# gareth-cross/mini_opt

Measured on AMD Instinct MI355X. Metric: batched dense KKT Newton steps/sec, n=64 fp64, higher is better.
Workload: dtype f64; 1 GPU; BASELINE configs[2]: batch=65536 per GPU, n=64 / 8 eq / 32 box, m_r=128, J-level input (row-major J), one mo_newton_step launch per step; mode=step, kernel=fused_mfma_f64_n64, batch_per_gpu=65536, batch_total=65536, n=64, k=8, m=32, m_r=128, parallelism=batch-sharded x1, no collectives

## Files before the change

### mini_opt_amd/csrc/kkt_fused.hip

```cpp
#include <math.h>
#include <stdlib.h>

#include <type_traits>

#include "mo_fused_device.h"
#include "mo_fused_diag.h"
#include "mo_fused_select.h"

namespace mo {
namespace {

typedef double d2 __attribute__((ext_vector_type(2)));
typedef double d4 __attribute__((ext_vector_type(4)));

constexpr int kRC = 15;

__device__ inline double readlane_f64(double v, int lane) {
  int lo = __double2loint(v), hi = __double2hiint(v);
  lo = __builtin_amdgcn_readlane(lo, lane);
  hi = __builtin_amdgcn_readlane(hi, lane);
  return __hiloint2double(hi, lo);
}
__device__ inline double bpermute_f64(int byte_addr, double v) {
  int lo = __builtin_amdgcn_ds_bpermute(byte_addr, __double2loint(v));
  int hi = __builtin_amdgcn_ds_bpermute(byte_addr, __double2hiint(v));
  return __hiloint2double(hi, lo);
}
typedef unsigned u2v __attribute__((ext_vector_type(2)));
template <int CTRL> __device__ inline double dpp_f64(double v) {
  int lo = __double2loint(v), hi = __double2hiint(v);
  lo = __builtin_amdgcn_mov_dpp(lo, CTRL, 0xf, 0xf, false);
  hi = __builtin_amdgcn_mov_dpp(hi, CTRL, 0xf, 0xf, false);
  return __hiloint2double(hi, lo);
}
__device__ inline double row_sum(double v) {
  v += dpp_f64<0xB1>(v);
  v += dpp_f64<0x4E>(v);
  v += dpp_f64<0x141>(v);
  v += dpp_f64<0x140>(v);
  return v;
}
__device__ inline int select_lanes32(unsigned long long mask, int if_set, int if_clear) {
  int r;
  asm("v_cndmask_b32 %0, %1, %2, %3" : "=v"(r) : "v"(if_clear), "v"(if_set), "s"(mask));
  return r;
}
__device__ inline double select_lanes(unsigned long long mask, double if_set, double if_clear) {
  return __hiloint2double(select_lanes32(mask, __double2hiint(if_set), __double2hiint(if_clear)),
                          select_lanes32(mask, __double2loint(if_set), __double2loint(if_clear)));
}
template <int CTRL, unsigned long long MASK> __device__ inline double exchange_add(double a, double b) {
  const double keep = select_lanes(MASK, b, a), send = select_lanes(MASK, a, b);
  return keep + dpp_f64<CTRL>(send);
}
__device__ inline double row_sum4_scatter(double p0, double p1, double p2, double p3) {
  const double q01 = exchange_add<0xB1, 0xAAAAAAAAAAAAAAAAull>(p0, p1);
  const double q23 = exchange_add<0xB1, 0xAAAAAAAAAAAAAAAAull>(p2, p3);
  double w = exchange_add<0x4E, 0xCCCCCCCCCCCCCCCCull>(q01, q23);
  w += dpp_f64<0x124>(w);
  w += dpp_f64<0x128>(w);
  return w;
}
__device__ inline double row_min(double v) {
  v = fmin(v, dpp_f64<0xB1>(v));
  v = fmin(v, dpp_f64<0x4E>(v));
  v = fmin(v, dpp_f64<0x141>(v));
  v = fmin(v, dpp_f64<0x140>(v));
  return v;
}
struct Rows2 { double a, b; };
__device__ inline Rows2 swap16_f64(double v) {
  const u2v lo = __builtin_amdgcn_permlane16_swap((unsigned)__double2loint(v), (unsigned)__double2loint(v), false, false);
  const u2v hi = __builtin_amdgcn_permlane16_swap((unsigned)__double2hiint(v), (unsigned)__double2hiint(v), false, false);
  return Rows2{__hiloint2double((int)hi[0], (int)lo[0]), __hiloint2double((int)hi[1], (int)lo[1])};
}
__device__ inline Rows2 swap32_f64(double v) {
  const u2v lo = __builtin_amdgcn_permlane32_swap((unsigned)__double2loint(v), (unsigned)__double2loint(v), false, false);
  const u2v hi = __builtin_amdgcn_permlane32_swap((unsigned)__double2hiint(v), (unsigned)__double2hiint(v), false, false);
  return Rows2{__hiloint2double((int)hi[0], (int)lo[0]), __hiloint2double((int)hi[1], (int)lo[1])};
}
__device__ inline double cross_row_sum(double v) {
  const Rows2 p = swap16_f64(v);
  const double s = p.a + p.b;
  const Rows2 q = swap32_f64(s);
  return q.a + q.b;
}
__device__ inline double cross_row_min(double v) {
  const Rows2 p = swap16_f64(v);
  const double s = fmin(p.a, p.b);
  const Rows2 q = swap32_f64(s);
  return fmin(q.a, q.b);
}
__device__ inline double rcp_f64(double d) {
  double q = __builtin_amdgcn_rcp(d);
  q = fma(q, fma(-d, q, 1.0), q);
  q = fma(q, fma(-d, q, 1.0), q);
  return q;
}
__device__ inline d4 mfma4(const d4& a, const d4& b, d4 c) {
  c = __builtin_amdgcn_mfma_f64_16x16x4f64(a[0], b[0], c, 0, 0, 0);
  c = __builtin_amdgcn_mfma_f64_16x16x4f64(a[1], b[1], c, 0, 0, 0);
  c = __builtin_amdgcn_mfma_f64_16x16x4f64(a[2], b[2], c, 0, 0, 0);
  c = __builtin_amdgcn_mfma_f64_16x16x4f64(a[3], b[3], c, 0, 0, 0);
  return c;
}

template <int NT, bool QPL> __device__ inline void ldv(const double* arr, int j, double (&v)[NT]) {
  if (QPL) {
#pragma unroll
    for (int c = 0; c < NT; ++c) v[c] = arr[16 * c + j];
  } else {
#pragma unroll
    for (int h = 0; h < NT / 2; ++h) { const d2 t = *(const d2*)(arr + 32 * h + 2 * j); v[2 * h] = t[0]; v[2 * h + 1] = t[1]; }
  }
}
template <int NT, bool QPL> __device__ inline void stv(double* arr, int j, const double (&v)[NT]) {
  if (QPL) {
#pragma unroll
    for (int c = 0; c < NT; ++c) arr[16 * c + j] = v[c];
  } else {
#pragma unroll
    for (int h = 0; h < NT / 2; ++h) { d2 t; t[0] = v[2 * h]; t[1] = v[2 * h + 1]; *(d2*)(arr + 32 * h + 2 * j) = t; }
  }
}
template <int NT, bool QPL> __device__ inline void ldv_n(const double* arr, int j, int nn, double (&v)[NT]) {
  if (QPL) {
#pragma unroll
    for (int c = 0; c < NT; ++c) v[c] = (16 * c + j < nn) ? arr[16 * c + j] : 0.0;
  } else {
#pragma unroll
    for (int h = 0; h < NT / 2; ++h) {
      v[2 * h] = (32 * h + 2 * j < nn) ? arr[32 * h + 2 * j] : 0.0;
      v[2 * h + 1] = (32 * h + 2 * j + 1 < nn) ? arr[32 * h + 2 * j + 1] : 0.0;
    }
  }
}
template <int NT, bool QPL> __device__ inline void stv_n(double* arr, int j, int nn, const double (&v)[NT]) {
  if (QPL) {
#pragma unroll
    for (int c = 0; c < NT; ++c)
      if (16 * c + j < nn) arr[16 * c + j] = v[c];
  } else {
#pragma unroll
    for (int h = 0; h < NT / 2; ++h) {
      if (32 * h + 2 * j < nn) arr[32 * h + 2 * j] = v[2 * h];
      if (32 * h + 2 * j + 1 < nn) arr[32 * h + 2 * j + 1] = v[2 * h + 1];
    }
  }
}
template <int NT, bool QPL> __device__ inline void pad_diag(int j, int nn, double (&v)[NT]) {
#pragma unroll
  for (int c = 0; c < NT; ++c) {
    const int nat = QPL ? 16 * c + j : 32 * (c >> 1) + 2 * j + (c & 1);
    v[c] = nat >= nn ? 1.0 : 0.0;
  }
}
template <int NT, bool QPL, int NY = 1>
__device__ inline void load_a_tiles(const double* Ap, int A_ld, int k, int nn, int g, int j, d4 (&U)[(NT + NY) * (NT + NY)]) {
  constexpr int NB = NT + NY;
  const int col_l = (QPL ? 1 : 2) * g;
  const double* Al = Ap + j + (size_t)col_l * A_ld;
#pragma unroll
  for (int c = 0; c < NT; ++c) {
#pragma unroll
    for (int t = 0; t < 4; ++t) {
      const int col_u = QPL ? (16 * c + 4 * t) : (32 * (c >> 1) + 8 * t + (c & 1));
#pragma unroll
      for (int q = 0; q < NY; ++q)
        U[c * NB + NT + q][t] = (16 * q + j < k && col_u + col_l < nn) ? Al[16 * q + (size_t)col_u * A_ld] : 0.0;
    }
  }
}
template <int NT, int NY = 1>
__device__ inline void load_g_tiles(const double* G, int ld, const double* cg, int nn, int g, int j, d4 (&U)[(NT + NY) * (NT + NY)],
                                    double (&cvec)[NT]) {
  constexpr int NB = NT + NY;
#pragma unroll
  for (int ta = 0; ta < NT; ++ta) {
#pragma unroll
    for (int tb = ta; tb < NT; ++tb) {
#pragma unroll
      for (int t = 0; t < 4; ++t) {
        const int r = g + 4 * t;
        int row = 16 * tb + j, col = 16 * ta + r;
        if (ta == tb && r > j) { row = 16 * ta + r; col = 16 * ta + j; }
        U[ta * NB + tb][t] = (row < nn && col < nn) ? G[row + (size_t)col * ld] : 0.0;
      }
    }
    cvec[ta] = (16 * ta + j < nn) ? cg[16 * ta + j] : 0.0;
  }
}

__device__ inline const void* uniform_ptr(const void* p) {
  return (const void*)(uintptr_t)uniform64((unsigned long long)(uintptr_t)p);
}
template <int IMM> __device__ inline void dma16_s(const void* sbase_in, unsigned voff, unsigned lds_dst_in) {
  const void* sbase = uniform_ptr(sbase_in);
  const unsigned lds_dst = __builtin_amdgcn_readfirstlane(lds_dst_in);
  unsigned keep;
  asm volatile(
      "s_mov_b32 %0, m0\n\ts_mov_b32 m0, %3\n\ts_nop 0\n\tglobal_load_lds_dwordx4 %1, %2 offset:%4 nt\n\ts_mov_b32 m0, %0"
      : "=&s"(keep)
      : "v"(voff), "s"(sbase), "s"(lds_dst), "i"(IMM)
      : "memory");
}
__device__ inline void dma4_s(const void* sbase_in, unsigned voff, unsigned lds_dst_in) {
  const void* sbase = uniform_ptr(sbase_in);
  const unsigned lds_dst = __builtin_amdgcn_readfirstlane(lds_dst_in);
  unsigned keep;
  asm volatile(
      "s_mov_b32 %0, m0\n\ts_mov_b32 m0, %3\n\ts_nop 0\n\tglobal_load_lds_dword %1, %2\n\ts_mov_b32 m0, %0"
      : "=&s"(keep)
      : "v"(voff), "s"(sbase), "s"(lds_dst)
      : "memory");
}
__device__ inline void dma_doubles(const double* src, unsigned lds_dst, int count, int lane) {
  const unsigned voff = 4u * (unsigned)lane;
  if (lane < 2 * count) dma4_s(src, voff, lds_dst);
  if (lane + 64 < 2 * count) dma4_s(reinterpret_cast<const char*>(src) + 256, voff, lds_dst + 256);
  if (count > 64) {
    if (lane + 128 < 2 * count) dma4_s(reinterpret_cast<const char*>(src) + 512, voff, lds_dst + 512);
    if (lane + 192 < 2 * count) dma4_s(reinterpret_cast<const char*>(src) + 768, voff, lds_dst + 768);
  }
  if (count > 128) {
#pragma unroll
    for (int c = 4; c < 8; ++c)
      if (lane + 64 * c < 2 * count) dma4_s(reinterpret_cast<const char*>(src) + 256 * c, voff, lds_dst + 256 * c);
  }
}

template <int LANE_IN_ROW> __device__ inline double row_bcast64(double v) {
  return __longlong_as_double(__builtin_amdgcn_mov_dpp(__double_as_longlong(v), 0x150 + LANE_IN_ROW, 0xf, 0xf, false));
}
template <unsigned long long MASK> __device__ inline void masked_set(double& dst, double src) {
  unsigned long long save;
  asm volatile("s_mov_b64 %[sv], exec\n\ts_mov_b32 exec_lo, %[lo]\n\ts_mov_b32 exec_hi, %[hi]\n\tv_mov_b64 %[d], %[s]\n\t"
               "s_mov_b64 exec, %[sv]\n\ts_nop 0"
               : [d] "+v"(dst), [sv] "=&s"(save)
               : [s] "v"(src), [lo] "i"((unsigned)(MASK & 0xffffffffull)), [hi] "i"((unsigned)(MASK >> 32)));
}
template <unsigned long long MASK> __device__ inline void masked_set_neg(double& dst, double src) {
  unsigned long long save;
  asm volatile("s_mov_b64 %[sv], exec\n\ts_mov_b32 exec_lo, %[lo]\n\ts_mov_b32 exec_hi, %[hi]\n\tv_max_f64 %[d], -%[s], -%[s]\n\t"
               "s_mov_b64 exec, %[sv]\n\ts_nop 0"
               : [d] "+v"(dst), [sv] "=&s"(save)
               : [s] "v"(src), [lo] "i"((unsigned)(MASK & 0xffffffffull)), [hi] "i"((unsigned)(MASK >> 32)));
}
template <unsigned long long MASK> __device__ inline void masked_zero4(d4& T) {
  unsigned long long save;
  double t0 = T[0], t1 = T[1], t2 = T[2], t3 = T[3];
  asm volatile(
      "s_mov_b64 %[sv], exec\n\ts_mov_b32 exec_lo, %[lo]\n\ts_mov_b32 exec_hi, %[hi]\n\tv_mov_b64 %[a], 0\n\tv_mov_b64 %[b], 0\n\t"
      "v_mov_b64 %[c], 0\n\tv_mov_b64 %[d], 0\n\ts_mov_b64 exec, %[sv]\n\ts_nop 0"
      : [a] "+v"(t0), [b] "+v"(t1), [c] "+v"(t2), [d] "+v"(t3), [sv] "=&s"(save)
      : [lo] "i"((unsigned)(MASK & 0xffffffffull)), [hi] "i"((unsigned)(MASK >> 32)));
  T[0] = t0; T[1] = t1; T[2] = t2; T[3] = t3;
}
template <int K>
__device__ inline void sweep_step_lean(d4& T, double& bad, int g, int j) {
  constexpr int src_g = K & 3, src_t = K >> 2;
  constexpr unsigned long long mcol = 0x0001000100010001ull << K;
  constexpr unsigned long long mrow = 0xFFFFull << (16 * src_g);
  const double rowreg = T[src_t];
  const double d = readlane_f64(rowreg, 16 * src_g + K);
  double inv = __builtin_amdgcn_rcp(d);
  inv = fma(inv, fma(-d, inv, 1.0), inv);
  asm volatile("v_fma_f64 %0, %1, 0, %0" : "+v"(bad) : "v"(inv));
  double rk = bpermute_f64((16 * src_g + j) * 4, rowreg) * inv;
  masked_set_neg<mcol>(rk, inv);
  double f[4];
#pragma unroll
  for (int t = 0; t < 4; ++t) f[t] = row_bcast64<K>(T[t]);
  masked_zero4<mcol>(T);
#pragma unroll
  for (int t = 0; t < 4; ++t) T[t] = fma(-f[t], rk, T[t]);
  double rowk_new = T[src_t];
  masked_set<mrow>(rowk_new, rk);
  T[src_t] = rowk_new;
}
template <int K, int KEND> struct SweepLoop {
  static __device__ inline void run(d4& T, double& bad, int npiv, int g, int j) {
    if (K < npiv) sweep_step_lean<K>(T, bad, g, j);
    SweepLoop<K + 1, KEND>::run(T, bad, npiv, g, j);
  }
};
template <int KEND> struct SweepLoop<KEND, KEND> {
  static __device__ inline void run(d4&, double&, int, int, int) {}
};
__device__ inline bool sweep_tile(d4& T, int npiv, int g, int j) {
  double bad = 0.0;
  SweepLoop<0, 16>::run(T, bad, npiv, g, j);
  return bad == 0.0;
}

template <int NT, int D, int JMODE = JMODE_VECTOR, int NY = 1, bool ROW0 = true, bool DIAG4 = false>
struct JStream {
  static constexpr bool FLAT = JMODE == JMODE_FLAT, GATHER = JMODE == JMODE_GATHER;
  static_assert(!DIAG4 || (JMODE == JMODE_VECTOR && NY == 1 && NT == 4), "DIAG4: the 16-byte stream of the 64 grid with one y tile");
  static constexpr int N = 16 * NT, NB = NT + NY, NH = NT / 2, NI = GATHER ? 2 * NT : (FLAT ? N / 8 : NH), DPS = NI + 1, SLOT = NH * 1024 + 64;
  static_assert((D - 1) * DPS <= 63, "vmcnt is a 6-bit counter");
  static_assert(D >= 2 && D <= 8, "ring depth");
  const char* jbase;
  const char* rbase;
  unsigned joff, roff;
  unsigned jstep;
  const double* tail_j; const double* tail_r; int rem, row_len, g_, j_;
  bool act0, act1, act2, act3;
  const char* lane_piece;
  const char* r_elem;
  const char* dop[DIAG4 ? diag4::kNumVec : 1];
  double dacc[DIAG4 ? NT / 2 : 1][diag4::kNumIns];
  unsigned ring_base;
  int lane, nsteps;
  long long rs_, cs_;

  __device__ inline void init(const double* Jp, const double* rg, const char* smem, unsigned ring_base_, int lane_, int g, int j, int m_r,
                              int nn = N, long long rs = -1, long long cs = 1) {
    if (rs < 0) rs = nn;
    jbase = reinterpret_cast<const char*>(Jp);
    rbase = reinterpret_cast<const char*>(rg);
    rs_ = 8 * rs; cs_ = 8 * cs;
    joff = GATHER ? (unsigned)(g * rs_ + 2 * j * cs_) : (unsigned)(g * nn + 2 * j) * 8u;
    jstep = GATHER ? (unsigned)(4 * rs_) : 32u * (unsigned)nn;
    act0 = 2 * j < nn; act1 = 32 + 2 * j < nn; act2 = 64 + 2 * j < nn; act3 = 96 + 2 * j < nn;
    roff = 4u * (unsigned)lane_;
    lane_piece = smem + lane_ * 16;
    if (DIAG4) {
      const int jp = diag4::swz(g, j);
      joff = (unsigned)(g * nn + 2 * jp) * 8u;
      act0 = 2 * jp < nn; act1 = 32 + 2 * jp < nn; act2 = 64 + 2 * jp < nn; act3 = 96 + 2 * jp < nn;
      lane_piece = smem + diag4::natural_off(lane_);
    }
    r_elem = smem + NH * 1024 + 8 * g;
    ring_base = ring_base_; lane = lane_; nsteps = m_r >> 2;
    rem = m_r & 3; row_len = nn; g_ = g; j_ = j;
    tail_j = Jp + (size_t)(4 * nsteps) * (GATHER ? rs : (long long)nn); tail_r = rg + 4 * nsteps;
  }
  template <int IMM> __device__ static inline void dma4_si(const void* sbase_in, unsigned voff, unsigned lds_dst_in) {
    const void* sbase = uniform_ptr(sbase_in);
    const unsigned lds_dst = __builtin_amdgcn_readfirstlane(lds_dst_in);
// ... 387 lines not shown
#pragma unroll
      for (int pb = pa + 1; pb < NB; ++pb) {
        double q2 = 0.0;
#pragma unroll
        for (int t = 0; t < 4; ++t) q2 = fma(U[pa * NB + pb][t], wr[t], q2);
        rb[pb] += cross_row_sum(q2);
        if constexpr (NY >= 2) asm volatile("" : "+v"(rb[pb]));
      }
      lds_fence();
    }
  }
#pragma unroll
  for (int pa = L; pa >= 0; --pa) {
    const double* rsrc = pa < NT ? rbuf_x + 16 * pa : rbuf_y + 16 * (pa - NT);
    double vt[4], pt[4];
#pragma unroll
    for (int t = 0; t < 4; ++t) {
      pt[t] = 0.0;
#pragma unroll
      for (int pb = pa + 1; pb < NB; ++pb) pt[t] = fma(U[pa * NB + pb][t], xb[pb], pt[t]);
    }
    if (pa < L) {
      const double ws = row_sum4_scatter(pt[0], pt[1], pt[2], pt[3]);
      pt[0] = row_bcast64<0>(ws); pt[1] = row_bcast64<1>(ws); pt[2] = row_bcast64<2>(ws); pt[3] = row_bcast64<3>(ws);
    }
#pragma unroll
    for (int t = 0; t < 4; ++t) vt[t] = rsrc[g + 4 * t] - pt[t];
    double q = 0.0;
#pragma unroll
    for (int t = 0; t < 4; ++t) q = fma(U[pa * NB + pa][t], vt[t], q);
    xb[pa] = -cross_row_sum(q);
    if (pa >= NT) xb[pa] = (16 * (pa - NT) + j < k) ? xb[pa] : 0.0;
    __builtin_amdgcn_sched_barrier(0);
  }
}

template <int NT, int WPS, int MC = 1, int NY = 1, bool RHS = false> struct FusedCfg {
  static constexpr int N = 16 * NT;
  static constexpr int NH = NT / 2;
  static constexpr int DPS = NH + 1;
  static constexpr int SLOT = NH * 1024 + 64;
  static constexpr int MCAP = 64 * MC;
  static constexpr int VEC = (3 * N + 4 * MCAP + MCAP / 2 + 32 * NY + (RHS ? MCAP : 0)) * 8;
  static constexpr int D_FIT = ((160 * 1024) / (4 * WPS) - VEC) / SLOT;
  static constexpr int D_TUNED = NT > 4 ? 4 : (NT == 4 ? (WPS >= 3 ? 4 : 7) : (WPS >= 4 ? 4 : 8));
  static constexpr int D = MC == 1 ? D_TUNED : (D_FIT > 8 ? 8 : D_FIT);
  static_assert(D >= 2, "LDS budget");
  static constexpr int LDS = D * SLOT + VEC;
};

template <int NT, int WPS, bool QPL, int MC = 1, int JMODE = JMODE_VECTOR, int NY = 1, bool RHS = false>
__global__ __launch_bounds__(256 * WPS, WPS) void kkt_fused_f64_kernel(const KernelArgs a) {
  static_assert(!RHS || JMODE == JMODE_VECTOR, "the right-hand-side mode exists on the 16-byte stream and for (G, c) only");
  using C = FusedCfg<NT, WPS, MC, NY, RHS>;
  constexpr int MCAP = C::MCAP;
  constexpr int N = C::N, NB = NT + NY, LT = NB - 1, SLOT = C::SLOT, D = C::D;
  constexpr int WAVES = 4 * WPS;

  __shared__ __attribute__((aligned(16))) char smem_all[WAVES * C::LDS];
  const int wave = __builtin_amdgcn_readfirstlane((int)(threadIdx.x >> 6));
  char* const smem = smem_all + wave * C::LDS;
  double* const xs = reinterpret_cast<double*>(smem + D * SLOT);
  double* const diagS = xs + N;
  double* const rhsS = diagS + N;
  double* const rp = diagS;
  double* const dxs = rhsS;
  double* const cA = rhsS + N;
  double* const cB = cA + MCAP;
  double* const cS = cB + MCAP;
  double* const cZ = cS + MCAP;
  int* const cV = reinterpret_cast<int*>(cZ + MCAP);
  double* const yb = cZ + MCAP + MCAP / 2;
  double* const bb = yb + 16 * NY;
  double* const cP = bb + 16 * NY;
  const unsigned ring_base = (unsigned)(uintptr_t)smem;
  const unsigned vec_base = ring_base + D * SLOT;

  const int m_lay = a.m;
  const bool no_ineq = (a.flags & MO_STEP_NO_INEQUALITIES) != 0;
  const int k = a.k, m = no_ineq ? 0 : a.m, m_r = a.m_r;
  const int nn = a.n;
  const bool transpose = RHS && (a.flags & MO_KKT_TRANSPOSE) != 0;
  constexpr bool DIAG4 = !RHS && !QPL && NT == 4 && NY == 1 && MC == 1 && JMODE == JMODE_VECTOR;
  if constexpr (DIAG4) {
    __builtin_assume(m <= MCAP);
    __builtin_assume(nn <= N);
    __builtin_assume(k <= 15);
  }
  for (int i = (int)(threadIdx.x & 63); i < D * SLOT / 8; i += 64) reinterpret_cast<double*>(smem)[i] = 0.0;
  for (int i = (int)(threadIdx.x & 63); i < N; i += 64) xs[i] = 0.0;
  lds_fence();
#ifdef MO_FUSED_STAMPS
  unsigned long long stamp_acc[16] = {0, 0, 0, 0, 0, 0, 0, 0, 0, 0, 0, 0, 0, 0, 0, 0}, stamp_prev;
  asm volatile("s_memtime %0\n\ts_waitcnt lgkmcnt(0)" : "=s"(stamp_prev)::"memory");
  const unsigned long long stamp_t0 = stamp_prev, stamp_rt0 = __builtin_amdgcn_s_memrealtime();
#endif

  const int chunk_shift = queue_chunk_shift<WAVES>();
  const long long waves_all = (long long)gridDim.x * WAVES;
  const bool st_rounds = a.static_rounds > 0 && a.batch <= (long long)a.static_rounds * waves_all;
  queue_stagger(a, st_rounds, wave);
  auto chunk_for = [&](long long observed) -> int {
    if (st_rounds) return 1;
    const long long c = (a.batch - observed) >> chunk_shift;
    return c < 1 ? 1 : (c > 8 ? 8 : (int)c);
  };
  int chunk = chunk_for(0);
  const long long ticket_base = (long long)gridDim.x * WAVES * chunk;
  long long p = st_rounds ? (long long)(wave >> 2) * ((long long)gridDim.x * 4) + (long long)blockIdx.x * 4 + (wave & 3) : ((long long)blockIdx.x * WAVES + wave) * chunk;
  long long chunk_end = p + chunk;

  while (p < a.batch) {
    const bool last_of_chunk = p + 1 >= chunk_end;
    int next_chunk = 0;
    unsigned long long next_ticket = 0;
    if (last_of_chunk) {
      next_chunk = chunk_for(p);
      next_ticket = queue_take_ticket(a, st_rounds, next_chunk, p);
    }
    const int lane = lane_id();
    const int g = lane >> 4, j = lane & 15;

    const double* Jp = QPL ? nullptr : (const double*)a.J + p * a.J_stride;
    const double* rg = QPL ? nullptr : RHS ? Jp : (const double*)a.r + p * a.r_stride;
    KArgs ka = fresh_args();
    const double* vp = (const double*)ka->vars + p * ka->vars_stride;
    const double* gp = RHS ? (const double*)ka->rhs + p * ka->rhs_stride : nullptr;

    JStream<NT, D, JMODE, NY, true, DIAG4> stream;
    if (!QPL) {
      stream.init(Jp, rg, smem, ring_base, lane, g, j, m_r, nn, a.J_row_major ? (long long)a.J_ld : 1ll, a.J_row_major ? 1ll : (long long)a.J_ld);
      stream.prologue();
    }
    MO_STAMP(13);

    d4 U[NB * NB];
#pragma unroll
    for (int q = 0; q < NB * NB; ++q) U[q] = d4{0.0, 0.0, 0.0, 0.0};
    dma_doubles(RHS ? gp : vp, vec_base, nn, lane);
    if (m > 0) {
      const long long coff = p * ka->cons_stride;
      if (lane < m) dma4_s(ka->cons_var + coff, 4u * (unsigned)lane, vec_base + (3 * N + 4 * MCAP) * 8);
#pragma unroll
      for (int ci = 1; ci < MC; ++ci)
        if (lane + 64 * ci < m) dma4_s(ka->cons_var + coff + 64 * ci, 4u * (unsigned)lane, vec_base + (3 * N + 4 * MCAP) * 8 + 256 * ci);
      dma_doubles((const double*)ka->cons_a + coff, vec_base + (3 * N) * 8, m, lane);
      if (RHS) {
        dma_doubles(gp + nn, vec_base + (3 * N + MCAP) * 8, m, lane);
        dma_doubles(gp + nn + m + k, vec_base + (3 * N + 4 * MCAP + MCAP / 2 + 32 * NY) * 8, m, lane);
      } else {
        dma_doubles((const double*)ka->cons_b + coff, vec_base + (3 * N + MCAP) * 8, m, lane);
      }
      dma_doubles(vp + nn, vec_base + (3 * N + 2 * MCAP) * 8, m, lane);
      dma_doubles(vp + nn + m + k, vec_base + (3 * N + 3 * MCAP) * 8, m, lane);
    }
    if (k > 0) {
      if (!RHS) dma_doubles(vp + nn + m_lay, vec_base + (3 * N + 4 * MCAP + MCAP / 2) * 8, k, lane);
      dma_doubles(RHS ? gp + nn + m_lay : (const double*)ka->b + p * ka->b_stride, vec_base + (3 * N + 4 * MCAP + MCAP / 2 + 16 * NY) * 8, k, lane);
    }
    MO_STAMP(14);
    load_a_tiles<NT, QPL, NY>(k > 0 ? (const double*)ka->A + p * ka->A_stride : nullptr, ka->A_ld, k, nn, g, j, U);

    MO_STAMP(0);
    double cpart[NT];
#pragma unroll
    for (int c = 0; c < NT; ++c) cpart[c] = 0.0;
    double cvec[NT];
    if (QPL) {
      load_g_tiles<NT, NY>((const double*)ka->G + p * ka->G_stride, ka->G_ld, (const double*)ka->c + p * ka->c_stride, nn, g, j, U, cvec);
    } else {
#ifdef MO_FUSED_STAMPS
      stream.wait_for_oldest(stream.nsteps - 1);
      MO_STAMP(7);
#endif
      stream.run(U, cpart);
      if constexpr (DIAG4) stream.diag_tiles(U, smem, nn < N);
#pragma unroll
      for (int c = 0; c < NT; ++c) cvec[c] = cross_row_sum(cpart[c]);
    }
    MO_STAMP(1);

    wait_vmcnt<0>();
    ka = fresh_args();
    const double mu = ka->mu ? ((const double*)ka->mu)[p * ka->mu_stride] : 0.0;
    if (lane < N / 2) {
      diagS[2 * lane] = 0.0; diagS[2 * lane + 1] = 0.0;
      rhsS[2 * lane] = 0.0; rhsS[2 * lane + 1] = 0.0;
    }
    int cvar[MC]; double ca[MC], cb[MC], cs[MC], cz[MC], cs_inv[MC];
    double cp[MC];
    bool bad_index[MC];
#pragma unroll
    for (int ci = 0; ci < MC; ++ci) {
      const int ix = lane + 64 * ci;
      cvar[ci] = 0; ca[ci] = 1.0; cb[ci] = 0.0; cs[ci] = 1.0; cz[ci] = 0.0; cp[ci] = 0.0;
      if (ix < m) { cvar[ci] = cV[ix]; ca[ci] = cA[ix]; cb[ci] = cB[ix]; cs[ci] = cS[ix]; cz[ci] = cZ[ix]; }
      if (RHS && ix < m) {
        cp[ci] = cP[ix];
        if (transpose) { cb[ci] = -(cs[ci] * cb[ci]); cB[ix] = cb[ci]; }
      }
    }
    lds_fence();
    bool lane_bad_slack = false, lane_bad_index = false;
#pragma unroll
    for (int ci = 0; ci < MC; ++ci) {
      const int ix = lane + 64 * ci;
      bad_index[ci] = (ix < m) && ((cvar[ci] < 0) || (cvar[ci] >= nn));
      if (bad_index[ci]) cvar[ci] = 0;
      lane_bad_index = lane_bad_index || bad_index[ci];
      lane_bad_slack = lane_bad_slack || ((ix < m) && !(cs[ci] > 0.0));
      cs_inv[ci] = rcp_f64(cs[ci]);
      if (ix < m) {
        const double zs = cz[ci] * cs_inv[ci];
        atomicAdd(&diagS[cvar[ci]], ca[ci] * zs * ca[ci]);
        if (RHS) atomicAdd(&rhsS[cvar[ci]], -(ca[ci] * (cb[ci] + cz[ci] * cp[ci]) * cs_inv[ci]));
        else atomicAdd(&rhsS[cvar[ci]], ca[ci] * (cz[ci] * (cs[ci] - cb[ci]) + mu) * cs_inv[ci]);
      }
    }
    const bool slack_bad = __any(lane_bad_slack);
    bool any_bad_index = __any(lane_bad_index);
    if (no_ineq && m_lay > 0) {
      bool bad = false;
      const int* cvp = ka->cons_var + p * ka->cons_stride;
      for (int ix = lane; ix < m_lay; ix += 64) { const int v = cvp[ix]; bad = bad || v < 0 || v >= nn; }
      any_bad_index = __any(bad);
    }
    lds_fence();
    double dS[NT], rS[NT];
    ldv<NT, QPL>(diagS, j, dS);
    ldv<NT, QPL>(rhsS, j, rS);
    if (RHS) {
      double rd[NT];
      ldv<NT, QPL>(xs, j, rd);
#pragma unroll
      for (int c = 0; c < NT; ++c) cvec[c] = transpose ? -rd[c] : rd[c];
    }
    if (g == 0) {
#pragma unroll
      for (int c = 0; c < NT; ++c) rp[16 * c + j] = rS[c] - cvec[c];
    }
    lds_fence();

#pragma unroll
    for (int t = 0; t < 4; ++t) {
      constexpr int e0 = 16 * (NY - 1);
      double v = 0.0;
      if (j == kRC) v = (e0 + g + 4 * t < k) ? -bb[e0 + g + 4 * t] : 0.0;
      if (g + 4 * t == kRC) v = (e0 + j < k) ? -bb[e0 + j] : 0.0;
      U[LT * NB + LT][t] = v;
#pragma unroll
      for (int q = 0; q < NY - 1; ++q) {
        if (j == kRC) U[(NT + q) * NB + LT][t] = -bb[16 * q + g + 4 * t];
      }
    }
    const double lam_in = ka->lambda_vec ? ((const double*)ka->lambda_vec)[p * ka->lambda_vec_stride] : ka->lambda;
    const double lam = (!QPL && lam_in > 0.0) ? lam_in : 0.0;
    double padv[NT];
    pad_diag<NT, QPL>(j, nn, padv);
#pragma unroll
    for (int c = 0; c < NT; ++c) {
#pragma unroll
      for (int t = 0; t < 4; ++t) {
        U[c * NB + c][t] += (j == g + 4 * t) ? (lam + dS[c] + padv[c]) : 0.0;
        const double rv = rp[16 * c + g + 4 * t];
        if (j == kRC) U[c * NB + LT][t] = rv;
      }
    }

    MO_STAMP(2);
    __builtin_amdgcn_sched_barrier(0);
    if (a.chain_prio) __builtin_amdgcn_s_setprio(1);
    bool ok = true;
    constexpr bool kLookAhead = NT >= kLookAheadMinNT && NY == 1;
    if constexpr (kLookAhead) {
      ok = block_eliminate_lookahead<NT>(U, k, g, j);
    } else {
#pragma unroll
    for (int pa = 0; pa < NB; ++pa) {
      ok = sweep_tile(U[pa * NB + pa], tile_pivots<NT, NY>(pa, k), g, j) && ok;
      __builtin_amdgcn_sched_barrier(0);
      MO_STAMP(3);
#pragma unroll
      for (int pc = pa + 1; pc < NB; ++pc) {
        d4 negZ = mfma4(U[pa * NB + pa], U[pa * NB + pc], d4{0.0, 0.0, 0.0, 0.0});
#pragma unroll
        for (int pb = pa + 1; pb <= pc; ++pb) U[pb * NB + pc] = mfma4(U[pa * NB + pb], negZ, U[pb * NB + pc]);
        __builtin_amdgcn_sched_barrier(0);
      }
      MO_STAMP(4);
    }
    }

    __builtin_amdgcn_sched_barrier(0);
    double xb[NB];
    back_substitute<NT, NY>(U, k, j, xb);

    MO_STAMP(5);
    ka = fresh_args();
    double dxv[NT];
    {
      double xn[NT];
      if (!RHS) ldv<NT, QPL>(xs, j, xn);
#pragma unroll
      for (int c = 0; c < NT; ++c) dxv[c] = RHS ? xb[c] : xb[c] - xn[c];
    }
    bool finite = true;
#pragma unroll
    for (int c = 0; c < NT; ++c) finite = finite && (fabs(dxv[c]) < INFINITY);
    if (g == 0) stv<NT, QPL>(dxs, j, dxv);
    lds_fence();
    double dsv[MC], dzv[MC], ap = 1.0, ad = 1.0;
#pragma unroll
    for (int ci = 0; ci < MC; ++ci) {
      const int ix = lane + 64 * ci;
      dsv[ci] = 0.0; dzv[ci] = 0.0;
      if (ix < m) {
        const double ca2 = cA[ix], cb2 = cB[ix], cs2 = cS[ix], cz2 = cZ[ix];
        const int cvar2 = bad_index[ci] ? 0 : cV[ix];
        const double csi = MC == 1 ? cs_inv[ci] : rcp_f64(cs2);
        if (RHS) {
          dsv[ci] = ca2 * dxs[cvar2] + cP[ix];
          dzv[ci] = -(cb2 + cz2 * dsv[ci]) * csi;
          finite = finite && (fabs(dsv[ci]) < INFINITY) && (fabs(dzv[ci]) < INFINITY);
          if (transpose) { dsv[ci] *= csi; dzv[ci] = -dzv[ci]; }
          continue;
        }
        const double r_pi = ca2 * xs[cvar2] + cb2 - cs2;
        dsv[ci] = ca2 * dxs[cvar2] + r_pi;
        dzv[ci] = -(cz2 * csi) * dsv[ci] - csi * (cs2 * cz2 - mu);
        const double tau = ka->tau;
        if (cs2 + dsv[ci] <= 0.0 && fabs(dsv[ci]) > 0.0) ap = fmin(ap, -tau * cs2 * rcp_f64(dsv[ci]));
        if (cz2 + dzv[ci] <= 0.0 && fabs(dzv[ci]) > 0.0) ad = fmin(ad, -tau * cz2 * rcp_f64(dzv[ci]));
        finite = finite && (fabs(dsv[ci]) < INFINITY) && (fabs(dzv[ci]) < INFINITY);
      }
    }
    if (!RHS) {
      ap = cross_row_min(row_min(ap));
      ad = cross_row_min(row_min(ad));
    }
    double dyv[NY];
#pragma unroll
    for (int q = 0; q < NY; ++q) {
      if (RHS) dyv[q] = (16 * q + j < k) ? (transpose ? xb[NT + q] : -xb[NT + q]) : 0.0;
      else dyv[q] = (16 * q + j < k) ? (-xb[NT + q] - yb[16 * q + j]) : 0.0;
      finite = finite && (fabs(dyv[q]) < INFINITY);
    }
    int st = MO_STATUS_OK;
    if (!__all(finite)) st = MO_STATUS_NONFINITE;
    if (!ok) st = MO_STATUS_FACTORIZATION_FAILED;
    if (slack_bad) st = MO_STATUS_NONPOSITIVE_SLACK;
    if (any_bad_index) st = MO_STATUS_BAD_INDEX;
    const double nanv = __builtin_nan("");
    double* dp = (double*)ka->delta + p * ka->delta_stride;
    if (g == 0) {
      double outv[NT];
#pragma unroll
      for (int c = 0; c < NT; ++c) outv[c] = st == MO_STATUS_OK ? dxv[c] : nanv;
      stv_n<NT, QPL>(dp, j, nn, outv);
#pragma unroll
      for (int q = 0; q < NY; ++q)
        if (16 * q + j < k) dp[nn + m_lay + 16 * q + j] = st == MO_STATUS_OK ? dyv[q] : nanv;
    }
    if (no_ineq) {
      for (int ix = lane; ix < m_lay; ix += 64) { dp[nn + ix] = st == MO_STATUS_OK ? 0.0 : nanv; dp[nn + m_lay + k + ix] = st == MO_STATUS_OK ? 0.0 : nanv; }
    }
#pragma unroll
    for (int ci = 0; ci < MC; ++ci) {
      const int ix = lane + 64 * ci;
      if (ix < m) {
        dp[nn + ix] = st == MO_STATUS_OK ? dsv[ci] : nanv;
        dp[nn + m + k + ix] = st == MO_STATUS_OK ? dzv[ci] : nanv;
      }
    }
    if (lane == 0) {
      if (!RHS && ka->alpha) {
        ((double*)ka->alpha)[2 * p] = st == MO_STATUS_OK ? ap : nanv;
        ((double*)ka->alpha)[2 * p + 1] = st == MO_STATUS_OK ? ad : nanv;
      }
      if (ka->status) ka->status[p] = st;
    }
    lds_fence();
    if (a.chain_prio) __builtin_amdgcn_s_setprio(0);
    MO_STAMP(6);
    if (last_of_chunk) { p = queue_ticket_problem(next_ticket, ticket_base); chunk_end = p + next_chunk; } else { ++p; }
  }
#ifdef MO_FUSED_STAMPS
  if ((threadIdx.x & 63) == 0 && a.debug) {
    for (int i = 0; i < 8; ++i) atomicAdd(a.debug + i, stamp_acc[i]);
    atomicAdd(a.debug + 13, stamp_acc[13]); atomicAdd(a.debug + 14, stamp_acc[14]);
    atomicAdd(a.debug + 8, 1ull);
    const unsigned long long life = stamp_prev - stamp_t0, rt = __builtin_amdgcn_s_memrealtime() - stamp_rt0;
    atomicMax(a.debug + 9, life);
    atomicMin(a.debug + 10, life);
    atomicAdd(a.debug + 11, rt);
    atomicMax(a.debug + 12, rt);
  }
#endif
}

template <int NT, int WPS, int JMODE = JMODE_VECTOR>
__global__ __launch_bounds__(256 * WPS, WPS) void kkt_fused_linearize_kernel(const KernelArgs a) {
  using C = FusedCfg<NT, WPS>;
  constexpr int NB = NT + 1, SLOT = C::SLOT, D = C::D;
  constexpr int WAVES = 4 * WPS;
  __shared__ __attribute__((aligned(16))) char smem_all[WAVES * C::LDS];
  const int wave = __builtin_amdgcn_readfirstlane((int)(threadIdx.x >> 6));
  char* const smem = smem_all + wave * C::LDS;
  const unsigned ring_base = (unsigned)(uintptr_t)smem;
  const int nn = a.n, m_r = a.m_r;
  for (int i = (int)(threadIdx.x & 63); i < D * SLOT / 8; i += 64) reinterpret_cast<double*>(smem)[i] = 0.0;
  lds_fence();
  const int chunk_shift = queue_chunk_shift<WAVES>();
  const long long waves_all = (long long)gridDim.x * WAVES;
  const bool st_rounds = a.static_rounds > 0 && a.batch <= (long long)a.static_rounds * waves_all;
  auto chunk_for = [&](long long observed) -> int {
    if (st_rounds) return 1;
    const long long c = (a.batch - observed) >> chunk_shift;
    return c < 1 ? 1 : (c > 8 ? 8 : (int)c);
  };
  int chunk = chunk_for(0);
  const long long ticket_base = (long long)gridDim.x * WAVES * chunk;
  long long p = st_rounds ? (long long)(wave >> 2) * ((long long)gridDim.x * 4) + (long long)blockIdx.x * 4 + (wave & 3) : ((long long)blockIdx.x * WAVES + wave) * chunk;
  long long chunk_end = p + chunk;
  while (p < a.batch) {
    const bool last_of_chunk = p + 1 >= chunk_end;
    int next_chunk = 0;
    unsigned long long next_ticket = 0;
    if (last_of_chunk) {
      next_chunk = chunk_for(p);
      next_ticket = queue_take_ticket(a, st_rounds, next_chunk, p);
    }
    const int lane = lane_id();
    const int g = lane >> 4, j = lane & 15;
    JStream<NT, D, JMODE> stream;
    stream.init((const double*)a.J + p * a.J_stride, (const double*)a.r + p * a.r_stride, smem, ring_base, lane, g, j, m_r, nn,
                a.J_row_major ? (long long)a.J_ld : 1ll, a.J_row_major ? 1ll : (long long)a.J_ld);
    stream.prologue();
    d4 U[NB * NB];
#pragma unroll
    for (int q = 0; q < NB * NB; ++q) U[q] = d4{0.0, 0.0, 0.0, 0.0};
    double cpart[NT];
#pragma unroll
    for (int c = 0; c < NT; ++c) cpart[c] = 0.0;
    stream.template run<true>(U, cpart);
    double cvec[NT];
#pragma unroll
    for (int c = 0; c < NT; ++c) cvec[c] = cross_row_sum(cpart[c]);
    const double half_sq = 0.5 * cross_row_sum(stream.rsq);
    const double lam_in = a.lambda_vec ? ((const double*)a.lambda_vec)[p * a.lambda_vec_stride] : a.lambda;
    const double lam = lam_in > 0.0 ? lam_in : 0.0;
    double* Go = (double*)a.G_out + p * a.G_out_stride;
    const int ld = a.G_out_ld;
    const bool whole_lines = NT <= 6 && nn == 16 * NT && !(ld & 1) && !(a.G_out_stride & 1) && (((uintptr_t)a.G_out & 15) == 0);
    if (whole_lines) {
      double* const stage = reinterpret_cast<double*>(smem);
      static_assert(D * SLOT >= 32 * 32 * 8, "the ring holds one 32 x 32 block");
#pragma unroll
      for (int sa = 0; sa < NT / 2; ++sa) {
#pragma unroll
        for (int sb = sa; sb < NT / 2; ++sb) {
          if (sa == sb) {
#pragma unroll
            for (int pq = 0; pq < 2; ++pq) {
// ... 897 lines not shown
```

Measured before the change: 48.59 million steps/s.

## Batch LDS fills and bordered-matrix setup with masked asm, pair alpha reductions

For vector-J configurations with at most four column tiles, constraint loads become unconditional and pinned, so LDS reads are issued together without branches. The bordered-system right-hand column is filled with exec-masked batched ds_read_b64, and diagonal regularization is applied with exec-masked adds instead of per-element selects. The two step-length minima (primal and dual) are reduced together through one permlane32 swap, and each half-wave writes one alpha. The intent is to cut VALU/select work and LDS latency in the per-problem setup and epilogue. The cost is reliance on padded constraint slots being readable past m and on hand-written inline asm correctness.

```diff
diff --git a/mini_opt_amd/csrc/kkt_fused.hip b/mini_opt_amd/csrc/kkt_fused.hip
--- a/mini_opt_amd/csrc/kkt_fused.hip
+++ b/mini_opt_amd/csrc/kkt_fused.hip
@@ -90,6 +90,13 @@
   const double s = fmin(p.a, p.b);
   const Rows2 q = swap32_f64(s);
   return fmin(q.a, q.b);
+}
+__device__ inline double wave_min_pair(double a, double b) {
+  const u2v lo = __builtin_amdgcn_permlane32_swap((unsigned)__double2loint(a), (unsigned)__double2loint(b), false, false);
+  const u2v hi = __builtin_amdgcn_permlane32_swap((unsigned)__double2hiint(a), (unsigned)__double2hiint(b), false, false);
+  const double s = fmin(__hiloint2double((int)hi[0], (int)lo[0]), __hiloint2double((int)hi[1], (int)lo[1]));
+  const Rows2 q = swap16_f64(s);
+  return row_min(fmin(q.a, q.b));
 }
 __device__ inline double rcp_f64(double d) {
   double q = __builtin_amdgcn_rcp(d);
@@ -256,6 +263,56 @@
       : [lo] "i"((unsigned)(MASK & 0xffffffffull)), [hi] "i"((unsigned)(MASK >> 32)));
   T[0] = t0; T[1] = t1; T[2] = t2; T[3] = t3;
 }
+template <unsigned long long MASK, int OFF> __device__ inline void masked_lds_read8(d4& A, d4& B, unsigned addr) {
+  unsigned long long save;
+  double a0 = A[0], a1 = A[1], a2 = A[2], a3 = A[3], b0 = B[0], b1 = B[1], b2 = B[2], b3 = B[3];
+  asm volatile(
+      "s_mov_b64 %[sv], exec\n\ts_mov_b32 exec_lo, %[lo]\n\ts_mov_b32 exec_hi, %[hi]\n\t"
+      "ds_read_b64 %[a0], %[ad] offset:%[o0]\n\tds_read_b64 %[a1], %[ad] offset:%[o1]\n\tds_read_b64 %[a2], %[ad] offset:%[o2]\n\t"
+      "ds_read_b64 %[a3], %[ad] offset:%[o3]\n\tds_read_b64 %[b0], %[ad] offset:%[o4]\n\tds_read_b64 %[b1], %[ad] offset:%[o5]\n\t"
+      "ds_read_b64 %[b2], %[ad] offset:%[o6]\n\tds_read_b64 %[b3], %[ad] offset:%[o7]\n\ts_mov_b64 exec, %[sv]\n\ts_waitcnt lgkmcnt(0)"
+      : [a0] "+v"(a0), [a1] "+v"(a1), [a2] "+v"(a2), [a3] "+v"(a3), [b0] "+v"(b0), [b1] "+v"(b1), [b2] "+v"(b2), [b3] "+v"(b3), [sv] "=&s"(save)
+      : [ad] "v"(addr), [o0] "i"(OFF), [o1] "i"(OFF + 32), [o2] "i"(OFF + 64), [o3] "i"(OFF + 96), [o4] "i"(OFF + 128), [o5] "i"(OFF + 160),
+        [o6] "i"(OFF + 192), [o7] "i"(OFF + 224), [lo] "i"((unsigned)(MASK & 0xffffffffull)), [hi] "i"((unsigned)(MASK >> 32))
+      : "memory");
+  A[0] = a0; A[1] = a1; A[2] = a2; A[3] = a3; B[0] = b0; B[1] = b1; B[2] = b2; B[3] = b3;
+}
+template <unsigned long long MASK> __device__ inline void masked_lds_read16(d4& A, d4& B, d4& C, d4& E, unsigned addr) {
+  unsigned long long save;
+  double a0 = A[0], a1 = A[1], a2 = A[2], a3 = A[3], b0 = B[0], b1 = B[1], b2 = B[2], b3 = B[3];
+  double c0 = C[0], c1 = C[1], c2 = C[2], c3 = C[3], e0 = E[0], e1 = E[1], e2 = E[2], e3 = E[3];
+  asm volatile(
+      "s_mov_b64 %[sv], exec\n\ts_mov_b32 exec_lo, %[lo]\n\ts_mov_b32 exec_hi, %[hi]\n\t"
+      "ds_read_b64 %[a0], %[ad]\n\tds_read_b64 %[a1], %[ad] offset:32\n\tds_read_b64 %[a2], %[ad] offset:64\n\tds_read_b64 %[a3], %[ad] offset:96\n\t"
+      "ds_read_b64 %[b0], %[ad] offset:128\n\tds_read_b64 %[b1], %[ad] offset:160\n\tds_read_b64 %[b2], %[ad] offset:192\n\tds_read_b64 %[b3], %[ad] offset:224\n\t"
+      "ds_read_b64 %[c0], %[ad] offset:256\n\tds_read_b64 %[c1], %[ad] offset:288\n\tds_read_b64 %[c2], %[ad] offset:320\n\tds_read_b64 %[c3], %[ad] offset:352\n\t"
+      "ds_read_b64 %[e0], %[ad] offset:384\n\tds_read_b64 %[e1], %[ad] offset:416\n\tds_read_b64 %[e2], %[ad] offset:448\n\tds_read_b64 %[e3], %[ad] offset:480\n\t"
+      "s_mov_b64 exec, %[sv]\n\ts_waitcnt lgkmcnt(0)"
+      : [a0] "+v"(a0), [a1] "+v"(a1), [a2] "+v"(a2), [a3] "+v"(a3), [b0] "+v"(b0), [b1] "+v"(b1), [b2] "+v"(b2), [b3] "+v"(b3),
+        [c0] "+v"(c0), [c1] "+v"(c1), [c2] "+v"(c2), [c3] "+v"(c3), [e0] "+v"(e0), [e1] "+v"(e1), [e2] "+v"(e2), [e3] "+v"(e3), [sv] "=&s"(save)
+      : [ad] "v"(addr), [lo] "i"((unsigned)(MASK & 0xffffffffull)), [hi] "i"((unsigned)(MASK >> 32))
+      : "memory");
+  A[0] = a0; A[1] = a1; A[2] = a2; A[3] = a3; B[0] = b0; B[1] = b1; B[2] = b2; B[3] = b3;
+  C[0] = c0; C[1] = c1; C[2] = c2; C[3] = c3; E[0] = e0; E[1] = e1; E[2] = e2; E[3] = e3;
+}
+template <unsigned long long MASK> __device__ inline void masked_add2(double& a, double va, double& b, double vb) {
+  unsigned long long save;
+  asm volatile(
+      "s_mov_b64 %[sv], exec\n\ts_mov_b32 exec_lo, %[lo]\n\ts_mov_b32 exec_hi, %[hi]\n\tv_add_f64 %[a], %[a], %[va]\n\tv_add_f64 %[b], %[b], %[vb]\n\t"
+      "s_mov_b64 exec, %[sv]\n\ts_nop 0"
+      : [a] "+v"(a), [b] "+v"(b), [sv] "=&s"(save)
+      : [va] "v"(va), [vb] "v"(vb), [lo] "i"((unsigned)(MASK & 0xffffffffull)), [hi] "i"((unsigned)(MASK >> 32)));
+}
+template <unsigned long long MASK> __device__ inline void masked_add4(double& a, double va, double& b, double vb, double& c, double vc, double& d, double vd) {
+  unsigned long long save;
+  asm volatile(
+      "s_mov_b64 %[sv], exec\n\ts_mov_b32 exec_lo, %[lo]\n\ts_mov_b32 exec_hi, %[hi]\n\tv_add_f64 %[a], %[a], %[va]\n\tv_add_f64 %[b], %[b], %[vb]\n\t"
+      "v_add_f64 %[c], %[c], %[vc]\n\tv_add_f64 %[d], %[d], %[vd]\n\ts_mov_b64 exec, %[sv]\n\ts_nop 0"
+      : [a] "+v"(a), [b] "+v"(b), [c] "+v"(c), [d] "+v"(d), [sv] "=&s"(save)
+      : [va] "v"(va), [vb] "v"(vb), [vc] "v"(vc), [vd] "v"(vd), [lo] "i"((unsigned)(MASK & 0xffffffffull)), [hi] "i"((unsigned)(MASK >> 32)));
+}
+__device__ inline void pin(double& v) { asm volatile("" : "+v"(v)); }
+__device__ inline void pin(int& v) { asm volatile("" : "+v"(v)); }
 template <int K>
 __device__ inline void sweep_step_lean(d4& T, double& bad, int g, int j) {
   constexpr int src_g = K & 3, src_t = K >> 2;
@@ -809,6 +866,7 @@
   const int nn = a.n;
   const bool transpose = RHS && (a.flags & MO_KKT_TRANSPOSE) != 0;
   constexpr bool DIAG4 = !RHS && !QPL && NT == 4 && NY == 1 && MC == 1 && JMODE == JMODE_VECTOR;
+  constexpr bool kBatchFills = NT <= 4 && JMODE == JMODE_VECTOR && NY <= 3;
   if constexpr (DIAG4) {
     __builtin_assume(m <= MCAP);
     __builtin_assume(nn <= N);
@@ -920,10 +978,16 @@
 #pragma unroll
     for (int ci = 0; ci < MC; ++ci) {
       const int ix = lane + 64 * ci;
-      cvar[ci] = 0; ca[ci] = 1.0; cb[ci] = 0.0; cs[ci] = 1.0; cz[ci] = 0.0; cp[ci] = 0.0;
-      if (ix < m) { cvar[ci] = cV[ix]; ca[ci] = cA[ix]; cb[ci] = cB[ix]; cs[ci] = cS[ix]; cz[ci] = cZ[ix]; }
+      if constexpr (kBatchFills) {
+        cvar[ci] = cV[ix]; ca[ci] = cA[ix]; cb[ci] = cB[ix]; cs[ci] = cS[ix]; cz[ci] = cZ[ix]; cp[ci] = RHS ? cP[ix] : 0.0;
+        pin(cvar[ci]); pin(ca[ci]); pin(cb[ci]); pin(cs[ci]); pin(cz[ci]);
+        if (RHS) pin(cp[ci]);
+      } else {
+        cvar[ci] = 0; ca[ci] = 1.0; cb[ci] = 0.0; cs[ci] = 1.0; cz[ci] = 0.0; cp[ci] = 0.0;
+        if (ix < m) { cvar[ci] = cV[ix]; ca[ci] = cA[ix]; cb[ci] = cB[ix]; cs[ci] = cS[ix]; cz[ci] = cZ[ix]; }
+        if (RHS && ix < m) cp[ci] = cP[ix];
+      }
       if (RHS && ix < m) {
-        cp[ci] = cP[ix];
         if (transpose) { cb[ci] = -(cs[ci] * cb[ci]); cB[ix] = cb[ci]; }
       }
     }
@@ -968,29 +1032,76 @@
     }
     lds_fence();
 
-#pragma unroll
-    for (int t = 0; t < 4; ++t) {
-      constexpr int e0 = 16 * (NY - 1);
-      double v = 0.0;
-      if (j == kRC) v = (e0 + g + 4 * t < k) ? -bb[e0 + g + 4 * t] : 0.0;
-      if (g + 4 * t == kRC) v = (e0 + j < k) ? -bb[e0 + j] : 0.0;
-      U[LT * NB + LT][t] = v;
-#pragma unroll
-      for (int q = 0; q < NY - 1; ++q) {
-        if (j == kRC) U[(NT + q) * NB + LT][t] = -bb[16 * q + g + 4 * t];
-      }
-    }
     const double lam_in = ka->lambda_vec ? ((const double*)ka->lambda_vec)[p * ka->lambda_vec_stride] : ka->lambda;
     const double lam = (!QPL && lam_in > 0.0) ? lam_in : 0.0;
     double padv[NT];
     pad_diag<NT, QPL>(j, nn, padv);
-#pragma unroll
-    for (int c = 0; c < NT; ++c) {
+    if constexpr (kBatchFills) {
+      constexpr unsigned long long kColRC = 0x0001000100010001ull << kRC;
+      double bcol[NY][4], brow = bb[16 * (NY - 1) + j];
 #pragma unroll
       for (int t = 0; t < 4; ++t) {
-        U[c * NB + c][t] += (j == g + 4 * t) ? (lam + dS[c] + padv[c]) : 0.0;
-        const double rv = rp[16 * c + g + 4 * t];
-        if (j == kRC) U[c * NB + LT][t] = rv;
+#pragma unroll
+        for (int q = 0; q < NY; ++q) bcol[q][t] = bb[16 * q + g + 4 * t];
+      }
+      const unsigned rp_row = vec_base + (N + g) * 8;
+      if constexpr (NT == 4) {
+        masked_lds_read16<kColRC>(U[LT], U[NB + LT], U[2 * NB + LT], U[3 * NB + LT], rp_row);
+      } else {
+#pragma unroll
+        for (int c = 0; c < NT; c += 2) masked_lds_read8<kColRC, 0>(U[c * NB + LT], U[(c + 1) * NB + LT], rp_row + 128 * c);
+      }
+#pragma unroll
+      for (int t = 0; t < 4; ++t) {
+        constexpr int e0 = 16 * (NY - 1);
+        double v = (j == kRC && e0 + g + 4 * t < k) ? -bcol[NY - 1][t] : 0.0;
+        if (t == 3) v = (g == 3) ? ((e0 + j < k) ? -brow : 0.0) : v;
+        U[LT * NB + LT][t] = v;
+#pragma unroll
+        for (int q = 0; q < NY - 1; ++q) {
+          double e = U[(NT + q) * NB + LT][t];
+          masked_set_neg<kColRC>(e, bcol[q][t]);
+          U[(NT + q) * NB + LT][t] = e;
+        }
+      }
+      double dadd[NT];
+#pragma unroll
+      for (int c = 0; c < NT; ++c) dadd[c] = lam + dS[c] + padv[c];
+#define MO_DIAG_ADD(t)                                                                                                                   \
+      {                                                                                                                                  \
+        constexpr unsigned long long md = 0x0008000400020001ull << (4 * t);                                                              \
+        double e[NT];                                                                                                                    \
+        _Pragma("unroll") for (int c = 0; c < NT; ++c) e[c] = U[c * NB + c][t];                                                          \
+        if constexpr (NT == 4) {                                                                                                         \
+          masked_add4<md>(e[0], dadd[0], e[1], dadd[1], e[2], dadd[2], e[3], dadd[3]);                                                   \
+        } else {                                                                                                                         \
+          _Pragma("unroll") for (int c = 0; c < NT; c += 2) masked_add2<md>(e[c], dadd[c], e[c + 1], dadd[c + 1]);                       \
+        }                                                                                                                                \
+        _Pragma("unroll") for (int c = 0; c < NT; ++c) U[c * NB + c][t] = e[c];                                                          \
+      }
+      MO_DIAG_ADD(0) MO_DIAG_ADD(1) MO_DIAG_ADD(2) MO_DIAG_ADD(3)
+#undef MO_DIAG_ADD
+    } else {
+#pragma unroll
+      for (int t = 0; t < 4; ++t) {
+        constexpr int e0 = 16 * (NY - 1);
+        double v = 0.0;
+        if (j == kRC) v = (e0 + g + 4 * t < k) ? -bb[e0 + g + 4 * t] : 0.0;
+        if (g + 4 * t == kRC) v = (e0 + j < k) ? -bb[e0 + j] : 0.0;
+        U[LT * NB + LT][t] = v;
+#pragma unroll
+        for (int q = 0; q < NY - 1; ++q) {
+          if (j == kRC) U[(NT + q) * NB + LT][t] = -bb[16 * q + g + 4 * t];
+        }
+      }
+#pragma unroll
+      for (int c = 0; c < NT; ++c) {
+#pragma unroll
+        for (int t = 0; t < 4; ++t) {
+          U[c * NB + c][t] += (j == g + 4 * t) ? (lam + dS[c] + padv[c]) : 0.0;
+          const double rv = rp[16 * c + g + 4 * t];
+          if (j == kRC) U[c * NB + LT][t] = rv;
+        }
       }
     }
 
@@ -1024,10 +1135,15 @@
 
     MO_STAMP(5);
     ka = fresh_args();
-    double dxv[NT];
+    double dxv[NT], ybv[NY];
+#pragma unroll
+    for (int q = 0; q < NY; ++q) ybv[q] = (kBatchFills && !RHS) ? yb[16 * q + j] : 0.0;
     {
       double xn[NT];
       if (!RHS) ldv<NT, QPL>(xs, j, xn);
+#pragma unroll
+      for (int q = 0; q < NY; ++q)
+        if (kBatchFills && !RHS) pin(ybv[q]);
 #pragma unroll
       for (int c = 0; c < NT; ++c) dxv[c] = RHS ? xb[c] : xb[c] - xn[c];
     }
@@ -1041,19 +1157,32 @@
     for (int ci = 0; ci < MC; ++ci) {
       const int ix = lane + 64 * ci;
       dsv[ci] = 0.0; dzv[ci] = 0.0;
+      double ca2 = 0.0, cb2 = 0.0, cs2 = 0.0, cz2 = 0.0, cp2 = 0.0, dxc = 0.0, xc = 0.0;
+      if constexpr (kBatchFills) {
+        ca2 = cA[ix]; cb2 = cB[ix]; cs2 = cS[ix]; cz2 = cZ[ix]; cp2 = RHS ? cP[ix] : 0.0;
+        int cvar2 = cV[ix];
+        pin(ca2); pin(cb2); pin(cs2); pin(cz2); pin(cvar2);
+        if (RHS) pin(cp2);
+        cvar2 = (unsigned)cvar2 < (unsigned)nn ? cvar2 : 0;
+        dxc = dxs[cvar2]; xc = RHS ? 0.0 : xs[cvar2];
+        pin(dxc);
+        if (!RHS) pin(xc);
+      } else if (ix < m) {
+        ca2 = cA[ix]; cb2 = cB[ix]; cs2 = cS[ix]; cz2 = cZ[ix]; cp2 = RHS ? cP[ix] : 0.0;
+        const int cvar2 = bad_index[ci] ? 0 : cV[ix];
+        dxc = dxs[cvar2]; xc = RHS ? 0.0 : xs[cvar2];
+      }
       if (ix < m) {
-        const double ca2 = cA[ix], cb2 = cB[ix], cs2 = cS[ix], cz2 = cZ[ix];
-        const int cvar2 = bad_index[ci] ? 0 : cV[ix];
         const double csi = MC == 1 ? cs_inv[ci] : rcp_f64(cs2);
         if (RHS) {
-          dsv[ci] = ca2 * dxs[cvar2] + cP[ix];
+          dsv[ci] = ca2 * dxc + cp2;
           dzv[ci] = -(cb2 + cz2 * dsv[ci]) * csi;
           finite = finite && (fabs(dsv[ci]) < INFINITY) && (fabs(dzv[ci]) < INFINITY);
           if (transpose) { dsv[ci] *= csi; dzv[ci] = -dzv[ci]; }
           continue;
         }
-        const double r_pi = ca2 * xs[cvar2] + cb2 - cs2;
-        dsv[ci] = ca2 * dxs[cvar2] + r_pi;
+        const double r_pi = ca2 * xc + cb2 - cs2;
+        dsv[ci] = ca2 * dxc + r_pi;
         dzv[ci] = -(cz2 * csi) * dsv[ci] - csi * (cs2 * cz2 - mu);
         const double tau = ka->tau;
         if (cs2 + dsv[ci] <= 0.0 && fabs(dsv[ci]) > 0.0) ap = fmin(ap, -tau * cs2 * rcp_f64(dsv[ci]));
@@ -1061,15 +1190,13 @@
         finite = finite && (fabs(dsv[ci]) < INFINITY) && (fabs(dzv[ci]) < INFINITY);
       }
     }
-    if (!RHS) {
-      ap = cross_row_min(row_min(ap));
-      ad = cross_row_min(row_min(ad));
-    }
+    double apd = 1.0;
+    if (!RHS) apd = wave_min_pair(ap, ad);
     double dyv[NY];
 #pragma unroll
     for (int q = 0; q < NY; ++q) {
       if (RHS) dyv[q] = (16 * q + j < k) ? (transpose ? xb[NT + q] : -xb[NT + q]) : 0.0;
-      else dyv[q] = (16 * q + j < k) ? (-xb[NT + q] - yb[16 * q + j]) : 0.0;
+      else dyv[q] = (16 * q + j < k) ? (-xb[NT + q] - (kBatchFills ? ybv[q] : yb[16 * q + j])) : 0.0;
       finite = finite && (fabs(dyv[q]) < INFINITY);
     }
     int st = MO_STATUS_OK;
@@ -1099,13 +1226,8 @@
         dp[nn + m + k + ix] = st == MO_STATUS_OK ? dzv[ci] : nanv;
       }
     }
-    if (lane == 0) {
-      if (!RHS && ka->alpha) {
-        ((double*)ka->alpha)[2 * p] = st == MO_STATUS_OK ? ap : nanv;
-        ((double*)ka->alpha)[2 * p + 1] = st == MO_STATUS_OK ? ad : nanv;
-      }
-      if (ka->status) ka->status[p] = st;
-    }
+    if (!RHS && ka->alpha && (lane & 31) == 0) ((double*)ka->alpha)[2 * p + (lane >> 5)] = st == MO_STATUS_OK ? apd : nanv;
+    if (lane == 0 && ka->status) ka->status[p] = st;
     lds_fence();
     if (a.chain_prio) __builtin_amdgcn_s_setprio(0);
     MO_STAMP(6);
```

Result: no change. 48.94 million steps/s (median of 6 runs) (+0.7%).
